# menonsamir/spiral

Measured on AMD Instinct MI355X. Metric: server ms/query + DB GB/s vs HBM roofline, 2^20 x 256B, lower is better.
Workload: dtype u32 residues, 32x32->64-bit integer MAC (two 28-bit CRT primes)

## Files before the change

### spiral_amd/csrc/digits_device.h

```cpp
#pragma once
#include <type_traits>

#include "common.h"
#include "ntt_device.h"

namespace spiral {

__device__ __forceinline__ uint64_t splitmix64(uint64_t x) {
    x += 0x9E3779B97F4A7C15ull;
    x = (x ^ (x >> 30)) * 0xBF58476D1CE4E5B9ull;
    x = (x ^ (x >> 27)) * 0x94D049BB133111EBull;
    return x ^ (x >> 31);
}

__device__ __forceinline__ uint64_t load_raw(const uint64_t* src, uint32_t idx, uint32_t tinv) {
    if (tinv == 0) return src[idx];
    uint32_t e = (idx * tinv) & (2 * kN - 1);
    uint64_t v = src[e & (kN - 1)];
    return (e & kN) ? kQ - v : v;
}

__device__ __forceinline__ uint64_t digit_of(uint64_t v, uint32_t k, uint32_t bits, uint64_t mask) {
    uint32_t sh = k * bits;
    if (bits <= 27u) {
// ... 12 lines not shown
    } else if (sh >= 32u) {
#pragma unroll
        for (int r = 0; r < 8; r++) d[r] = (hi32(raw[r]) >> (sh - 32u)) & mask;
    } else {
#pragma unroll
        for (int r = 0; r < 8; r++) d[r] = __builtin_amdgcn_alignbit(hi32(raw[r]), lo32(raw[r]), sh) & mask;
    }
}
__device__ __forceinline__ uint32_t udiv_small(uint32_t b, uint32_t d, uint32_t inv) { return d == 1u ? b : __umulhi(b, inv); }

template <bool SMALL>
__device__ __forceinline__ uint32_t digit_residue(uint32_t d, uint32_t m) {
    if constexpr (SMALL) return d;
    return d < (1u << 28) ? d : d % m;
}
constexpr uint32_t kSmallDigitBits = 27;
#define DIGIT_WIDTH_DISPATCH(bits, body) \
    do {                                 \
        if ((bits) <= kSmallDigitBits)   \
            body(std::true_type{});      \
        else                             \
            body(std::false_type{});     \
    } while (0)

struct SDigit {
    uint32_t sh_chain, sh_digit;
    uint64_t low_mask, thresh_in;
    uint64_t mask, base, thresh;
    bool has_in, may;
};
__device__ __forceinline__ SDigit sdigit_setup(uint32_t k, uint32_t bits, uint32_t ell) {
    SDigit d;
    const uint32_t half = ell >> 1, start = k < half ? 0u : half, j = k - start;
    d.base = 1ull << bits;
    d.mask = d.base - 1;
    d.thresh = d.base >> 1;
    d.sh_chain = start * bits;
    d.sh_digit = k * bits;
    d.has_in = j > 0;
    d.low_mask = (bits * j >= 64) ? ~0ull : ((1ull << (bits * j)) - 1);
    uint64_t t = 0;
    for (uint32_t i = 0; i < j; i++) t = (t << bits) + d.thresh;
    d.thresh_in = t;
    d.may = k < half ? (k + 1 < half) : true;
    return d;
}
// ... 139 lines not shown
```

### spiral_amd/csrc/kernels.h

```cpp
#pragma once
#include <hip/hip_runtime.h>
#include <stdint.h>
#include <stdlib.h>

#include <atomic>

#include "common.h"

namespace spiral {

struct IndexMap {
    uint32_t inner, outer_stride, off;
    __host__ __device__ uint32_t operator()(uint32_t b) const { return (b / inner) * outer_stride + (b % inner) + off; }
};
inline IndexMap identity_map() { return IndexMap{1u, 1u, 0u}; }

#ifdef SPIRAL_TUNING
inline const char* tuning_env(const char* name) { return getenv(name); }
#else
inline const char* tuning_env(const char*) { return nullptr; }
#endif
struct Options {
    int fold_pair = 1, fold_chain = 1, fwd2 = -1;
    uint32_t fold_blocks = 768, sweep_mfma_min = 2, fwd2_min = 8192;
    size_t db_stage_bytes = (size_t)64 << 20;
    int one_image = 1;
    uint32_t pack_item_group = 0;
    uint32_t pack_batch_lanes = 0;
    int pack_pair_blocks = 0;
    int sweep_narrow = 0;
    uint32_t query_batch_chunk = 512;
};
Options& options();

#ifndef SPIRAL_MAX_LANES
#define SPIRAL_MAX_LANES 8
#endif
constexpr uint32_t kMaxLanes = SPIRAL_MAX_LANES;
struct Lanes {
    uint32_t n = 1;
    int64_t off[kMaxLanes] = {};
#ifdef __HIPCC__
    __device__ __forceinline__ int64_t here() const {
        const uint32_t z = blockIdx.z;
        int64_t o = 0;
#pragma unroll
        for (uint32_t q = 1; q < kMaxLanes; q++) o = z == q ? off[q] : o;
        return o;
    }
    __device__ __forceinline__ int64_t at(int64_t stride) const { return (int64_t)blockIdx.z * stride; }
#endif
};
#ifdef __HIPCC__
// ... 228 lines not shown
void launch_response_wire_slots(const uint64_t* in, uint64_t* out, uint32_t n0, uint32_t w0, uint32_t n1, uint32_t w1, const Slots& slots, int64_t out_stride,
                                hipStream_t s);

struct ExpandMacParamsCore {
    uint64_t* cv;
    const uint64_t* w_e;
    const uint64_t* w_o;
    const uint64_t* g;
    const uint64_t* a1;
    uint32_t cnt_e, cnt_o, t_e, t_o;
    ExpandActive act;
    const uint64_t* neg1n;
    const uint64_t* neg1ns;
    uint32_t next_num_in, next_cnt_o;
};
template <class L>
struct ExpandMacParamsT : ExpandMacParamsCore {
    using Core = ExpandMacParamsCore;
    using NoLanesT = ExpandMacParamsT<NoLanes>;
    L lanes;
};
using ExpandMacParams = ExpandMacParamsT<Lanes>;
void launch_expand_mac_round(const ExpandMacParams& p, hipStream_t s);
struct Scal2MatParamsCore {
    const uint64_t* w;
    const uint64_t* g;
    const uint64_t* cv;
    IndexMap cv_pos;
    uint64_t* out;
    uint32_t* qs;
    uint32_t t_conv, count, jm_total, j_base;
};
template <class L>
struct Scal2MatParamsT : Scal2MatParamsCore {
    using Core = Scal2MatParamsCore;
    using NoLanesT = Scal2MatParamsT<NoLanes>;
    L lanes;
};
using Scal2MatParams = Scal2MatParamsT<Lanes>;
void launch_scal2mat(const Scal2MatParams& p, hipStream_t s);
struct GswParamsCore {
    const uint64_t* w;
    const uint64_t* v;
    const uint64_t* chat;
    const uint64_t* cv;
    IndexMap cv_pos;
// ... 244 lines not shown
```

### spiral_amd/csrc/ntt.hip

```cpp
#include <algorithm>
#include <cstdio>
#include <cstdlib>
#include <type_traits>

#include "digits_device.h"
#include "kernels.h"
#include "ntt_device.h"
#include "wire_device.h"

namespace spiral {

__device__ __forceinline__ void pk_load8_red(const uint64_t* poly, bool reduce, uint32_t tid, uint32_t* lo, uint32_t* hi) {
    uint64_t x[8];
    pk_load8(poly, tid, x);
    pk_unpack8(x, lo, hi);
    if (reduce) {
#pragma unroll
        for (int r = 0; r < 8; r++) {
            lo[r] %= kP;
            hi[r] %= kB;
        }
    }
}

// ... 46 lines not shown
                *p.err = 1u;
                v %= p.p_db;
            }
            if (v >= half_p) {
                uint64_t d = p.p_db - v;
                lo[r] = kP - mod_p(d);
                hi[r] = kB - mod_b(d);
            } else {
                lo[r] = mod_p(v);
                hi[r] = mod_b(v);
            }
        }
    } else if constexpr (LOAD == LD_PDIGIT) {
        uint32_t sp;
        if (p.pmode == PM_GSW) {
            sp = s;
        } else if (p.pmode == PM_FOLD) {
            const uint32_t per_t = 4u * p.fold_np, t = s / per_t, rem = s - t * per_t;
            sp = (t * p.pk_num_per + (rem >> 1)) * 2u + (rem & 1u);
        } else {
            sp = s * p.pk_num_per * 2u;
        }
        const uint64_t* src = p.src + (size_t)sp * kN;
        const uint64_t mask = (1ull << p.bits) - 1;
        uint64_t raw[8];
#pragma unroll
        for (int r = 0; r < 8; r++) raw[r] = src[ix_a(tid, r)];
        if (p.bits <= kSmallDigitBits) {
            udigits8(raw, k, p.bits, lo);
#pragma unroll
            for (int r = 0; r < 8; r++) hi[r] = lo[r];
        } else {
#pragma unroll
            for (int r = 0; r < 8; r++) {
                uint32_t d = (uint32_t)digit_of(raw[r], k, p.bits, mask);
                lo[r] = digit_residue<false>(d, kP);
                hi[r] = digit_residue<false>(d, kB);
            }
        }
    } else if constexpr (LOAD == LD_EXPAND) {
        const uint32_t je = p.cnt_e * p.t_e;
        uint32_t a, tdim;
        if (b < je) {
            tdim = p.t_e;
            a = udiv_small(b, tdim, p.inv_te);
            k = b - a * tdim;
        } else {
            tdim = p.t_o;
            const uint32_t bb = b - je;
            a = udiv_small(bb, tdim, p.inv_to);
            k = bb - a * tdim;
            a += p.cnt_e;
        }
        const uint64_t* src = p.src + (size_t)a * 2u * kN;
        uint64_t raw[8];
#pragma unroll
        for (int r = 0; r < 8; r++) raw[r] = src[ix_a(tid, r)];
        const uint32_t bits = get_bits_per(tdim);
        if (bits <= kSmallDigitBits) {
            udigits8(raw, k, bits, lo);
#pragma unroll
            for (int r = 0; r < 8; r++) hi[r] = lo[r];
        } else {
            const uint64_t mask = (1ull << bits) - 1;
#pragma unroll
            for (int r = 0; r < 8; r++) {
                const uint32_t d = (uint32_t)digit_of(raw[r], k, bits, mask);
                lo[r] = digit_residue<false>(d, kP);
                hi[r] = digit_residue<false>(d, kB);
            }
        }
        s = b;
    } else if constexpr (LOAD == LD_SDIFF) {
        const uint32_t i = s / 6u, rc = s - i * 6u;
        const uint64_t* sl = p.src + ((size_t)i * 6u + rc) * kN;
        const uint64_t* sh_ = p.src + ((size_t)(p.fold_np + i) * 6u + rc) * kN;
        const SFast f = sfast_setup(k, p.bits, p.ell);
        if (f.ok && (!f.chain1 || f.x_hi)) {
            const uint32_t* wl = reinterpret_cast<const uint32_t*>(sl) + (f.chain1 ? 1u : 0u);
            const uint32_t* wh = reinterpret_cast<const uint32_t*>(sh_) + (f.chain1 ? 1u : 0u);
            uint32_t xl[8], xh[8];
#pragma unroll
            for (int r = 0; r < 8; r++) {
                xl[r] = wl[2u * ix_a(tid, r)];
                xh[r] = wh[2u * ix_a(tid, r)];
            }
            const uint32_t xs = f.chain1 ? f.x_sh : 0u;
            if (f.last0) {
#pragma unroll
                for (int r = 0; r < 8; r++) signed_residues((int32_t)(sfast_word<true>(xh[r], f) - sfast_word<true>(xl[r], f)), lo[r], hi[r]);
            } else if (xs == 0u) {
#pragma unroll
                for (int r = 0; r < 8; r++) signed_residues((int32_t)(sfast_word<false>(xh[r], f) - sfast_word<false>(xl[r], f)), lo[r], hi[r]);
            } else {
// ... 570 lines not shown
```

### spiral_amd/csrc/poly.hip

```cpp
#include <cstdlib>
#include <type_traits>
#include "common.h"
#include "kernels.h"

namespace spiral {

__device__ __forceinline__ uint32_t shoup32(uint32_t y, uint32_t w, uint32_t ws, uint32_t m) { return w * y - __umulhi(y, ws) * m; }

constexpr uint32_t kTpb = 256;
constexpr uint32_t kBpp = kN / kTpb;

struct Acc2 {
    uint64_t lo = 0, hi = 0;
    __device__ __forceinline__ void mac(uint64_t a, uint64_t b) {
        lo += (uint64_t)lo32(a) * lo32(b);
        hi += (uint64_t)hi32(a) * hi32(b);
    }
    __device__ __forceinline__ uint64_t reduced() const { return pack(mod_p(lo), mod_b(hi)); }
};
__device__ __forceinline__ uint64_t add_pk(uint64_t a, uint64_t b) {
    return pack(csub(lo32(a) + lo32(b), kP), csub(hi32(a) + hi32(b), kB));
}

template <class L>
__global__ __launch_bounds__(kTpb) void matmul_kernel(MatmulParamsT<L> p) {
    const uint32_t z = blockIdx.x * kTpb + threadIdx.x;
    uint32_t rc = blockIdx.y, bt = blockIdx.z;
    if constexpr (!std::is_same<L, NoLanes>::value) {
        const int64_t lane = p.lanes.here();
        lane_shift(p.a, lane);
        lane_shift(p.b, lane);
        lane_shift(p.out, lane);
        bt = blockIdx.y / (p.rs * p.cs);
        rc = blockIdx.y - bt * (p.rs * p.cs);
    }
    const uint32_t r = rc / p.cs, c = rc - r * p.cs;
    const uint64_t* a = p.a + ((size_t)bt * p.a_batch + (size_t)r * p.ms) * kN + z;
    const uint64_t* b = p.b + ((size_t)bt * p.b_batch + c) * kN + z;
    Acc2 acc;
    for (uint32_t m = 0; m < p.ms; m++) acc.mac(a[(size_t)m * kN], b[(size_t)m * p.cs * kN]);
    p.out[((size_t)bt * p.out_batch + rc) * kN + z] = acc.reduced();
}
void launch_matmul(const MatmulParams& p, uint32_t batch, hipStream_t s) {
    if (batch == 0) return;
    if (p.lanes.n > 1)
// ... 1000 lines not shown
```

### spiral_amd/csrc/primitives.cpp

```cpp
#include "server_state.h"

thread_local std::string spiral::host::g_err;
std::atomic<uint64_t> spiral::host::g_pack_lane_batches{0};
std::atomic<uint64_t> spiral::g_mfma_sweeps{0};
std::atomic<uint64_t> spiral::host::g_db_export_ns{0};

spiral::Options& spiral::options() {
    static Options o = [] {
        Options v;
        if (const char* e = getenv("SPIRAL_FOLD_PAIR")) v.fold_pair = atoi(e) != 0;
        if (const char* e = getenv("SPIRAL_SWEEP_MFMA")) v.sweep_mfma_min = (uint32_t)strtoul(e, nullptr, 10);
        if (const char* e = getenv("SPIRAL_DB_STAGE_BYTES")) v.db_stage_bytes = (size_t)strtoull(e, nullptr, 10);
        return v;
    }();
    return o;
}

namespace {
size_t base_message_bytes(const spiral_gpu_params* p, MessageLayout (*layout)(const spiral_gpu_params&, const spiral_gpu_shape&), Form form) {
    spiral_gpu_shape s;
    return shape_of(p, &s) ? 0 : message_bytes(layout(*p, s), form);
}
}

extern "C" {

int spiral_gpu_abi_version(void) { return SPIRAL_GPU_ABI_VERSION; }

int spiral_gpu_set_option(const char* name, int64_t value) {
    if (!name) return fail("null option name");
    Options& o = options();
    const std::string n = name;
    if (n == "fold_pair") o.fold_pair = value != 0;
    else if (n == "fold_chain") o.fold_chain = value != 0;
    else if (n == "fold_blocks" && value >= 0) o.fold_blocks = (uint32_t)value;
    else if (n == "sweep_mfma_min" && value >= 0) o.sweep_mfma_min = (uint32_t)value;
    else if (n == "one_image") o.one_image = value != 0;
    else if (n == "fwd2" && value >= -1 && value <= 1) o.fwd2 = (int)value;
    else if (n == "fwd2_min" && value >= 0) o.fwd2_min = (uint32_t)value;
    else if (n == "db_stage_bytes" && value > 0) o.db_stage_bytes = (size_t)value;
    else if (n == "pack_item_group" && value >= 0 && value <= 0xFFFFFFFFll) o.pack_item_group = (uint32_t)value;
    else if (n == "pack_batch_lanes" && value >= 0 && value <= (int64_t)kMaxLanes) o.pack_batch_lanes = (uint32_t)value;
    else if (n == "pack_pair_blocks" && (value == 0 || value == 1)) o.pack_pair_blocks = (int)value;
    else if (n == "sweep_narrow" && (value == 0 || value == 1)) o.sweep_narrow = (int)value;
    else if (n == "query_batch_chunk" && value >= 1 && value <= 0xFFFFFFFFll) o.query_batch_chunk = (uint32_t)value;
    else return fail("unknown option '%s' or value %lld out of range", name, (long long)value);
    return 0;
}
int spiral_gpu_get_option(const char* name, int64_t* value) {
    if (!name || !value) return fail("null argument");
    const Options& o = options();
    const std::string n = name;
    if (n == "fold_pair") *value = o.fold_pair;
    else if (n == "fold_chain") *value = o.fold_chain;
    else if (n == "fold_blocks") *value = o.fold_blocks;
    else if (n == "sweep_mfma_min") *value = o.sweep_mfma_min;
    else if (n == "one_image") *value = o.one_image;
    else if (n == "fwd2") *value = o.fwd2;
    else if (n == "fwd2_min") *value = o.fwd2_min;
    else if (n == "db_stage_bytes") *value = (int64_t)o.db_stage_bytes;
    else if (n == "pack_item_group") *value = o.pack_item_group;
    else if (n == "pack_batch_lanes") *value = o.pack_batch_lanes;
    else if (n == "pack_pair_blocks") *value = o.pack_pair_blocks;
    else if (n == "sweep_narrow") *value = o.sweep_narrow;
    else if (n == "query_batch_chunk") *value = o.query_batch_chunk;
    else if (n == "graph_captures") *value = (int64_t)g_captures.load();
    else if (n == "pack_lane_batches") *value = (int64_t)g_pack_lane_batches.load();
    else if (n == "key_binds") *value = (int64_t)g_key_binds.load();
    else if (n == "db_export_ns") *value = (int64_t)g_db_export_ns.load();
    else if (n == "mfma_sweeps") *value = (int64_t)g_mfma_sweeps.load(std::memory_order_relaxed);
    else return fail("unknown option '%s'", name);
    return 0;
}
const char* spiral_gpu_last_error(void) { return g_err.c_str(); }
int spiral_gpu_device_count(void) {
    int n = 0;
    if (hipGetDeviceCount(&n) != hipSuccess) return 0;
    return n;
}
int spiral_gpu_get_shape(const spiral_gpu_params* p, spiral_gpu_shape* out) { return shape_of(p, out); }
int spiral_gpu_has_limb_form(const spiral_gpu_params* p, uint32_t j_begin, uint32_t j_end) {
    if (!p) return fail("null argument");
    spiral_gpu_shape s;
    spiral_gpu_params q = *p;
    q.direct_upload = 1;
    if (shape_of(&q, &s)) return -1;
    if (j_end == 0 && j_begin == 0) j_end = s.dim0;
    if (j_begin >= j_end || j_end > s.dim0) return fail("bad first-dimension shard [%u, %u) of %u", j_begin, j_end, s.dim0);
    return DbLayout::base(s.num_per, j_end - j_begin).limbs_ok() ? 1 : 0;
}
int spiral_gpu_column_shard_has_limb_form(const spiral_gpu_params* p, uint32_t n_ranks) {
    if (!p) return fail("null argument");
    spiral_gpu_shape s;
// ... 428 lines not shown
```

### spiral_amd/csrc/server.cpp

```cpp
#include "records_host.h"
#include "server_state.h"

std::atomic<uint64_t> spiral::host::g_captures{0};

namespace {

uint32_t fold_dpb(const spiral_gpu_server* S, uint32_t n_src) {
    uint32_t dpb = S->s.ell;
    while (dpb > 1 && n_src * ((S->s.ell + dpb - 1) / dpb) < S->fold_blocks) dpb = (dpb + 1) / 2;
    return dpb;
}

int srv_alloc(spiral_gpu_server* S, DbImage* owners) {
    const spiral_gpu_params& p = S->p;
    const spiral_gpu_shape& s = S->s;
    S->img = owners ? owners->share() : DbImage::create(DbLayout::base(srv_np(S), S->dim0_shard), S);
    if (!S->img) return -1;
    S->n_cv = p.direct_upload ? s.n_bits : (1u << s.g);
    const size_t ngs = (size_t)p.nu2 * s.ell;
    const size_t half = s.num_per > 1 ? s.num_per / 2 : 1;
    auto layout = [&](Arena& a) {
        a.carve(S->w_left, (size_t)s.n_left * 2 * p.t_exp * kN);
        a.carve(S->w_right, (size_t)s.n_right * 2 * p.t_exp_right * kN);
        a.carve(S->w, (size_t)3 * 2 * p.t_conv * kN);
// ... 162 lines not shown
    if (n_ii == 0 || ii0 >= S->s.num_per || n_ii > S->s.num_per - ii0) return fail("column range out of bounds");
    const size_t per_z = (size_t)n_ii * 2 * S->dim0_shard * 2;
    const uint32_t zchunk = (uint32_t)std::max<size_t>(1, std::min<size_t>(nz, ((size_t)256 << 20) / (per_z * sizeof(uint64_t))));
    DevBuf st;
    if (st.alloc(per_z * zchunk)) return -1;
    hipError_t e = hipSuccess;
    for (uint32_t z = 0; z < nz && e == hipSuccess; z += zchunk) {
        const uint32_t n = std::min(zchunk, nz - z);
        launch_db_read_slots(S->img->db.p, st.p, S->s.num_per, S->dim0_shard, z_begin + z, n, ii0, n_ii, S->stream, S->img->format == SPIRAL_GPU_DB_LIMBS);
        e = hipMemcpyAsync(out + (size_t)z * per_z, st.p, (size_t)n * per_z * sizeof(uint64_t), hipMemcpyDeviceToHost, S->stream);
        if (e == hipSuccess) e = hipStreamSynchronize(S->stream);
    }
    st.release();
    if (e != hipSuccess) return fail("database read-back failed: %s", hipGetErrorString(e));
    return 0;
}
}

namespace spiral {
namespace host {

void srv_check_epoch(spiral_gpu_server* S) {
    const uint64_t e = S->img->epoch;
    if (S->epoch_seen != e) {
        srv_drop_graphs(S);
        S->epoch_seen = e;
    }
}

int sweep_mfma(const uint64_t* limbs, const uint32_t* const* qs, uint64_t* const* acc, uint32_t n, uint32_t np, uint32_t jm, uint32_t g_log, hipStream_t st,
               uint32_t k_log, uint32_t g_extra) {
    const hipError_t e = launch_sweep_mfma(limbs, qs, acc, n, np, jm, g_log, st, k_log, g_extra);
    return e == hipSuccess ? 0 : fail("the matrix-core sweep could not be launched: %s", hipGetErrorString(e));
}
int sweep_one(spiral_gpu_server* S, int stage) {
    const DbImage* H = S->img;
    if (H->format == SPIRAL_GPU_DB_LIMBS) {
        if (stage >= 0 && S->sweep_k_log)
            return fail("a staged sweep needs the packed database image, and a batch has since converted it to limb planes: call set_sweep_stages again (or set option one_image = 0)");
        const uint32_t* qs[1] = {(const uint32_t*)S->qs.p};
        uint64_t* acc[1] = {S->acc};
        return sweep_mfma(H->db.p, qs, acc, 1, srv_np(S), 2 * S->dim0_shard, sweep_g_log(S), S->stream, S->sweep_k_log);
    }
    launch_sweep(H->db.p, (const uint32_t*)S->qs.p, S->acc, srv_np(S), 2 * S->dim0_shard, sweep_g_log(S), S->stream, S->sweep_k_log, stage);
    return 0;
}

int srv_join_side(spiral_gpu_server* S) {
    if (S->side_pending) {
        HIP_OK(hipStreamWaitEvent(S->stream, S->ev_join, 0));
// ... 4 lines not shown

void mark_raw_stale(spiral_gpu_server* const* servers, uint32_t n) {
    for (uint32_t b = 0; b < n; b++) servers[b]->raw_from_acc = false;
}
void mark_swept(spiral_gpu_server* const* servers, uint32_t n) {
    for (uint32_t b = 0; b < n; b++) servers[b]->have_records = true;
    mark_raw_stale(servers, n);
}

int expand_lanes(spiral_gpu_server* S, const Lanes& lanes, uint32_t r_begin, uint32_t r_end) {
    const spiral_gpu_params& p = S->p;
    if (p.direct_upload || S->s.g == 0) {
        const size_t n = p.direct_upload ? (size_t)S->s.n_bits * 2 : 2;
        for (uint32_t q = 0; q < lanes.n && r_begin == 0; q++)
            HIP_OK(hipMemcpyAsync(S->cv.p + lanes.off[q], S->query.p + lanes.off[q], n * kPolyBytes, hipMemcpyDeviceToDevice, S->stream));
        return 0;
    }
    ExpandWork wk{S->ex_raw.p, S->ex_g.p};
    run_expand(S->tb, S->cv.p, S->s.g, p.t_exp, S->w_left.p, p.t_exp_right, S->w_right.p, S->s.ell * p.nu2, S->s.stopround, wk, S->stream, S->query.p, r_begin, r_end,
               S->ex_shard, 3, lanes);
    return 0;
}

int convert_part(spiral_gpu_server* S, uint32_t what, hipStream_t st, bool mark_split, const Lanes& lanes) {
    const spiral_gpu_params& p = S->p;
    const spiral_gpu_shape& s = S->s;
    const uint32_t ps = S->pos_stride, ngs = p.nu2 * s.ell;
    if (ngs == 0) what &= ~CONV_GSW;
    if (what & CONV_S2M) S->have_records = true;
    const uint32_t n1 = (what & CONV_S2M) ? S->dim0_shard : 0, n2 = (what & CONV_GSW) ? 2 * ngs : 0;
    const IndexMap map1{1, 2 * ps, 2 * (S->j0 * ps + S->pos_first)};
    const IndexMap map2{2, 2 * ps, 2 * S->pos_rest};
    uint64_t* raw = n1 ? S->cv_raw.p : S->gs_raw_p;
    launch_job(S->tb, lift_job(S->cv.p, raw, n1 + n2, {.src_map = n1 ? map1 : map2, .split = (n1 && n2) ? n1 : 0, .src_map2 = map2, .lanes = lanes}), st);
    launch_job(S->tb, gadget_digits_job(raw, n1 ? S->cv_g.p : S->gs_chat_p, n1 + n2, p.t_conv, 2 * p.t_conv, lanes), st);
    Scal2MatParams sp{};
    sp.w = S->w.p;
    sp.g = S->cv_g.p;
    sp.cv = S->cv.p;
    sp.cv_pos = IndexMap{1, ps, S->j0 * ps + S->pos_first};
    sp.out = S->keep_cts ? S->cts_keep.p : nullptr;
    sp.qs = (uint32_t*)S->qs.p;
    sp.t_conv = p.t_conv;
    sp.count = S->dim0_shard;
    sp.jm_total = 2 * S->dim0_shard;
    sp.j_base = 0;
    sp.lanes = lanes;
    GswParams gp{};
    gp.w = S->w.p;
    gp.v = S->v.p;
    gp.chat = S->gs_chat_p;
    gp.cv = S->cv.p;
    gp.cv_pos = IndexMap{1, ps, S->pos_rest};
    gp.gsw = S->key.p;
    gp.t_conv = p.t_conv;
    gp.ell = s.ell;
    gp.dims = p.nu2;
    gp.key = nullptr;
    gp.lanes = lanes;
    if (what == CONV_BOTH && !mark_split) {
        launch_convert_products(sp, gp, st);
        return 0;
    }
    if (what & CONV_S2M) launch_scal2mat(sp, st);
    if (mark_split) HIP_OK(hipEventRecord(S->ev[7], st));
    if (what & CONV_GSW) launch_regev_to_gsw(gp, st);
    return 0;
}

int expand_convert(spiral_gpu_server* S) {
    if (expand_lanes(S, Lanes{})) return -1;
    return convert_part(S, CONV_BOTH, S->stream, !S->use_graphs);
}

int finish_lanes(spiral_gpu_server* S, const Lanes& lanes) {
    launch_rescale2(S->raw.p, S->resp.p, 2 * kN, 6 * kN, kQ, S->s.qprime, 4 * S->p.p_db, S->stream, lanes);
    return 0;
}
int run_fold_rounds(spiral_gpu_server* S, const FoldJob& job) {
    const spiral_gpu_shape& s = S->s;
    const Lanes& lanes = job.lanes;
    S->raw_from_acc = false;
    uint32_t np = job.np0;
    const uint64_t *src_pk = job.src_pk, *raw_addend = job.raw_addend;
    bool pre_reduce = job.pre_reduce;
    auto lift = [&](uint32_t npolys) {
        launch_job(S->tb, lift_job(src_pk, S->raw.p, npolys, {.pre_reduce = pre_reduce, .lanes = lanes}), S->stream);
        src_pk = nullptr;
    };
    auto digits = [&](FwdLoad ld, uint32_t n_src, uint32_t mac_terms) {
        launch_job(S->tb, fold_digits_job(ld, S->raw.p, S->fold_d.p, n_src, s.ell, np, mac_terms, lanes), S->stream);
    };
    uint64_t* out_pk = S->fold_c.p;
    for (uint32_t d = job.d0; d < job.d0 + job.rounds; d++) {
        np /= 2;
// ... 555 lines not shown
}

int spiral_gpu_server_run_pre(spiral_gpu_server* S) {
    if (enter(S)) return -1;
    if (!S->have_query || !S->have_pp) return fail("query and public parameters must be set first");
    const spiral_gpu_params& p = S->p;
    auto half = [&](uint32_t parity, hipStream_t st, uint64_t* raw, uint64_t* g) {
        ExpandWork wk{raw, g};
        run_expand(S->tb, S->cv.p, S->s.g, p.t_exp, S->w_left.p, p.t_exp_right, S->w_right.p, S->s.ell * p.nu2, S->s.stopround, wk, st, S->query.p, 0, 0xffffffffu,
                   ExpandShard{}, parity);
    };
    if (S->overlap) {
        if (srv_join_side(S)) return -1;
        HIP_OK(hipEventRecord(S->ev_fork, S->stream));
        HIP_OK(hipStreamWaitEvent(S->side_stream, S->ev_fork, 0));
        if (run_graph(S, G_PRE_SIDE, S->side_stream, {}, [&]() {
                half(2u, S->side_stream, S->ex_raw2.p, S->ex_g2.p);
                return convert_part(S, CONV_GSW, S->side_stream);
            }))
            return -1;
        HIP_OK(hipEventRecord(S->ev_join, S->side_stream));
        S->side_pending = true;
    }
    if (int rc = run_graph(S, G_PRE, S->stream, {}, [&]() {
            if (!S->overlap) return expand_convert(S);
            half(1u, S->stream, S->ex_raw.p, S->ex_g.p);
            return convert_part(S, CONV_S2M, S->stream);
        }))
        return rc;
    S->have_records = true;
    return 0;
}

int spiral_gpu_server_run_query(spiral_gpu_server* S) {
    if (enter(S)) return -1;
    if (refuse_column(S, "run_query")) return -1;
    if (!S->have_query || !S->have_pp) return fail("query and public parameters must be set first");
    if (!S->img->loaded) return fail("no database loaded");
    if (S->overlap) {
        if (spiral_gpu_server_run_pre(S)) return -1;
        if (spiral_gpu_server_first_dim(S)) return -1;
        return spiral_gpu_server_run_post(S, 0);
    }
    if (srv_join_side(S)) return -1;
    if (int rc = run_graph(S, G_QUERY, S->stream, {}, [&]() {
            if (expand_convert(S)) return -1;
            if (spiral_gpu_server_first_dim(S)) return -1;
            return run_fold_rounds(S, {.np0 = S->s.num_per, .rounds = S->p.nu2, .src_pk = S->acc, .finish = true});
        }))
        return rc;
    mark_swept(&S, 1);
    return 0;
}

int spiral_gpu_server_fold_local(spiral_gpu_server* S, const void* acc_chunk, void* out_ct) {
    if (!S || !acc_chunk || !out_ct) return fail("null argument");
    if (refuse_column(S, "fold_local")) return -1;
    HIP_OK(hipSetDevice(S->device));
    const uint32_t L = S->s.num_per >> S->fold_g_log;
    if (srv_join_side(S)) return -1;
    if (int rc = run_graph(S, G_FOLD_LOCAL, S->stream, {word(acc_chunk), word(out_ct)}, [&]() {
            if (run_fold_rounds(S, {.np0 = L, .rounds = S->p.nu2 - S->fold_g_log, .src_pk = (const uint64_t*)acc_chunk, .pre_reduce = true})) return -1;
            HIP_OK(hipMemcpyAsync(out_ct, S->raw.p, 6 * kPolyBytes, hipMemcpyDeviceToDevice, S->stream));
            return 0;
        }))
        return rc;
    S->raw_from_acc = false;
    return 0;
}

int spiral_gpu_server_fold_root(spiral_gpu_server* S, const void* gathered_cts) {
    if (!S || !gathered_cts) return fail("null argument");
    HIP_OK(hipSetDevice(S->device));
    const uint32_t G = 1u << S->fold_g_log;
    if (srv_join_side(S)) return -1;
    if (int rc = run_graph(S, G_FOLD_ROOT, S->stream, {word(gathered_cts)}, [&]() {
            HIP_OK(hipMemcpyAsync(S->raw.p, gathered_cts, (size_t)G * 6 * kPolyBytes, hipMemcpyDeviceToDevice, S->stream));
            return run_fold_rounds(S, {.np0 = G, .d0 = S->p.nu2 - S->fold_g_log, .rounds = S->fold_g_log, .finish = true});
        }))
        return rc;
    S->raw_from_acc = false;
    return 0;
}

int spiral_gpu_server_run_pre_sweep(spiral_gpu_server* S) {
    if (enter(S)) return -1;
    if (refuse_column(S, "run_pre_sweep")) return -1;
    if (!S->have_query || !S->have_pp) return fail("query and public parameters must be set first");
    if (!S->img->loaded) return fail("no database loaded");
    if (S->overlap) {
        if (spiral_gpu_server_run_pre(S)) return -1;
        return spiral_gpu_server_first_dim(S);
    }
    if (int rc = run_graph(S, G_PRE_SWEEP, S->stream, {}, [&]() {
            if (expand_convert(S)) return -1;
            return spiral_gpu_server_first_dim(S);
        }))
        return rc;
    mark_swept(&S, 1);
    return 0;
}

int spiral_gpu_server_run_expand_pack(spiral_gpu_server* S, void* bits_out) {
    if (!S || !bits_out) return fail("null argument");
    if (refuse_column(S, "run_expand_pack")) return -1;
    HIP_OK(hipSetDevice(S->device));
    if (!S->have_query || !S->have_pp) return fail("query and public parameters must be set first");
    return run_graph(S, G_EXPAND_PACK, S->stream, {word(bits_out)}, [&]() {
        if (expand_lanes(S, Lanes{})) return -1;
        return spiral_gpu_server_gsw_bits_pack(S, bits_out);
    });
}

int spiral_gpu_server_run_unpack_convert_sweep(spiral_gpu_server* S, const void* gathered) {
    if (!S || !gathered) return fail("null argument");
    if (refuse_column(S, "run_unpack_convert_sweep")) return -1;
    HIP_OK(hipSetDevice(S->device));
    if (!S->img->loaded) return fail("no database loaded");
    if (int rc = run_graph(S, G_UNPACK_CONVERT_SWEEP, S->stream, {word(gathered)}, [&]() {
            if (spiral_gpu_server_gsw_bits_unpack(S, gathered)) return -1;
            if (convert_part(S, CONV_BOTH, S->stream, !S->use_graphs)) return -1;
// ... 216 lines not shown
```

### spiral_amd/csrc/server_lanes.cpp

```cpp
#include "server_state.h"

namespace {

int check_lanes(spiral_gpu_server* const* servers, uint32_t n, const char* what, uint32_t needs, Lanes* lanes) {
    const bool whole = !(needs & SWEEP_ONLY), sharded = needs & SHARDED, moves = needs & MOVES_DATA;
    const bool column_ok = needs & (COLUMN_SHARDS | COLUMN_ONLY | MOVES_DATA | GIVES_KEYS | SWEEP_ONLY);
    return check_lane_list(servers, n, what, needs, lanes, [&](uint32_t b) {
        const spiral_gpu_server *S = servers[0], *L = servers[b];
        if (L->col.on && !column_ok) return refuse_column(L, what);
        if ((needs & COLUMN_ONLY) && !L->col.on) return fail("%s: server %u is not a column shard (create_column_shard)", what, b);
        if (!(L->col == S->col))
            return fail("%s: server %u is %s, server 0 %s: the lanes of a call are column shards of one rank and rank count, or none is", what, b,
                        L->col.on ? "a column shard of another rank or rank count" : "no column shard", S->col.on ? "is a column shard" : "is none");
        if (whole && (((needs & NEED_QUERY) && !L->have_query) || (!L->have_pp && !(needs & (GIVES_KEYS | MOVES_DATA))))) return fail("%s: server %u needs its query and public parameters set first", what, b);
        if ((needs & NEED_DB) && !L->img->loaded) return fail("%s: server %u has no database", what, b);
        if ((needs & NEED_RECORDS) && !L->have_records) return fail("%s: server %u has not converted its query (run_pre first)", what, b);
        if (L->device != S->device || L->dim0_shard != S->dim0_shard || L->s.num_per != S->s.num_per ||
            (whole && (memcmp(&L->p, &S->p, sizeof(S->p)) != 0 || L->j0 != S->j0 || L->j1 != S->j1)))
            return fail("%s: server %u differs from server 0 in parameters, device or shard", what, b);
        if ((sharded || !whole) && L->fold_g_log != S->fold_g_log)
            return fail("%s: server %u has %u fold ranks, server 0 has %u", what, b, 1u << L->fold_g_log, 1u << S->fold_g_log);
        if (sharded && (L->ex_shard.g_log != S->ex_shard.g_log || L->ex_shard.rank != S->ex_shard.rank))
            return fail("%s: server %u has another expansion shard than server 0", what, b);
        if (whole && !sharded && !moves && (L->acc != L->acc_own.p || (L->fold_g_log && !L->col.on) || L->ex_shard.g_log))
// ... 347 lines not shown
            if (sweep_image(S->img, limbs, qs, acc, n, 0, S->stream)) return -1;
            return run_fold_rounds(S, {.np0 = S->s.num_per, .rounds = S->p.nu2, .src_pk = S->acc, .finish = true, .lanes = lanes});
        });
    if (!rc) mark_swept(servers, n);
    return rc;
}

int spiral_gpu_server_run_query_instances(spiral_gpu_server* S, spiral_gpu_server* const* instances, uint32_t n, int pre, void* responses, void* finals) {
    if (!S || !instances || n == 0 || !responses) return fail("null argument");
    Lanes one;
    if (check_lanes(&S, 1, "run_query_instances", NEED_QUERY | (pre ? 0 : NEED_RECORDS), &one)) return -1;
    if (check_instances(S, instances, n, "run_query_instances")) return -1;
    std::vector<uint64_t> key{word(responses), word(finals), pre != 0};
    key_instances(&key, instances, n, nullptr);
    if (srv_join_side(S)) return -1;
    ItemOut o;
    o.resp = (uint64_t*)responses;
    o.fin = (uint64_t*)finals;
    o.via_resp = true;
    auto body = [&]() {
        if (pre && expand_convert(S)) return -1;
        return item_rounds(&S, Lanes{}, instances, nullptr, n, o);
    };
    if (int rc = run_graph(S, G_INSTANCES, S->stream, key, body)) return rc;
    if (pre)
        mark_swept(&S, 1);
    else
        mark_raw_stale(&S, 1);
    return 0;
}

int spiral_gpu_server_answer_instances(spiral_gpu_server* S, spiral_gpu_server* const* instances, uint32_t n, const uint64_t* query, uint64_t* responses,
                                       uint64_t* finals, double* total_us) {
    if (!S || !instances || n == 0 || !query || !responses) return fail("null argument");
    if (refuse_column(S, "answer_instances")) return -1;
    HIP_OK(hipSetDevice(S->device));
    if (spiral_gpu_server_set_query(S, query)) return -1;
    const size_t bytes = (size_t)n * 6 * kPolyBytes;
    return answer_on_host(S, {responses, bytes}, {finals, bytes}, total_us,
                          [&](void* d_resp, void* d_fin) { return spiral_gpu_server_run_query_instances(S, instances, n, 1, d_resp, d_fin); });
}

int spiral_gpu_server_run_query_batch_instances(spiral_gpu_server* const* servers, uint32_t n, spiral_gpu_server* const* instances, uint32_t n_inst, int pre,
                                                void* responses, void* finals, void* wire) {
    Lanes lanes;
    if (!responses && !wire) return fail("run_query_batch_instances: no output (responses or wire)");
    if (check_batch_instances(servers, n, instances, n_inst, pre, true, &lanes)) return -1;
// ... 189 lines not shown
```

### spiral_amd/csrc/server_state.h

```cpp
#pragma once
#include "db_image.h"
#include "key_store.h"
#include "message.h"

using namespace spiral;
using namespace spiral::host;

enum GraphId : int {
    G_PRE = 0,
    G_POST = 1,
    G_POST_REDUCE = 2,
    G_PRE_SIDE = 3,
    G_QUERY = 4,
    G_FOLD_LOCAL = 5,
    G_FOLD_ROOT = 6,
    G_PRE_SWEEP = 7,
    G_EXPAND_PACK = 8,
    G_UNPACK_CONVERT_SWEEP = 9,
    G_SCAL2MAT_SWEEP = 10,
    G_UNPACK_GSW = 11,
    G_SCAL2MAT = 12,
    G_BATCH,
    G_INSTANCES,
    G_BATCH_INSTANCES,
// ... 32 lines not shown
    DevBuf w_left, w_right, w, v, query, cv, ex_raw, ex_g, ex_raw2, ex_g2;
    DevBuf cv_raw, cv_g, key, cts_keep;
    uint64_t *gs_raw_p = nullptr, *gs_chat_p = nullptr;
    DevBuf qs, acc_own, raw, fold_d, fold_c, fold_c2, resp, stage;
    WireIn wire_in;
    QueryBatchIn query_batch_in;
    KeyMemo key_memo;
    uint64_t* acc = nullptr;
    hipEvent_t ev[8] = {};
    bool use_graphs = false;
    Captured graphs[G_COUNT];
    int overlap = 0;
    bool side_pending = false;
    hipStream_t side_stream = nullptr;
    hipEvent_t ev_fork = nullptr, ev_join = nullptr;
    bool fold_chain = true;
    bool fold_pair = true;
    uint32_t fold_blocks = 768;
    uint32_t fold_g_log = 0;
    uint32_t sweep_k_log = 0;
    ExpandShard ex_shard{};
    uint32_t sweep_mfma_min = 2;
    uint64_t epoch_seen = 0;
};

namespace spiral {
namespace host {

extern std::atomic<uint64_t> g_captures;

struct FoldJob {
    uint32_t np0 = 0, d0 = 0, rounds = 0;
    const uint64_t* src_pk = nullptr;
    bool pre_reduce = false, finish = false;
    const uint64_t* raw_addend = nullptr;
    Lanes lanes{};
};
enum ConvertWhat : uint32_t { CONV_S2M = 1, CONV_GSW = 2, CONV_BOTH = 3 };

constexpr uint32_t kMinShardColumns = 1;
inline uint32_t column_shard_columns(uint32_t num_per, uint32_t rank, uint32_t n_ranks) {
    if (n_ranks == 0 || (n_ranks & (n_ranks - 1))) return fail("column shards: %u ranks, the rank count must be a power of two", n_ranks), 0u;
    if (num_per / n_ranks < kMinShardColumns)
        return fail("column shards: %u ranks leave %u of %u ciphertext columns per shard, a shard needs at least %u", n_ranks, num_per / n_ranks, num_per,
                    kMinShardColumns),
               0u;
    if (rank >= n_ranks) return fail("column shard %u of %u: no such rank", rank, n_ranks), 0u;
    return num_per / n_ranks;
}
inline uint32_t srv_np(const spiral_gpu_server* S) { return S->s.num_per >> (S->col.on ? S->col.g_log : 0u); }
inline uint32_t col_g_log(const spiral_gpu_server* S) { return S->col.on ? S->col.g_log : 0u; }
inline uint32_t col_ranks(const spiral_gpu_server* S) { return 1u << col_g_log(S); }
inline bool holds_column(const spiral_gpu_server* S, uint32_t ii) { return (ii & (col_ranks(S) - 1u)) == (S->col.on ? S->col.rank : 0u); }
inline uint32_t sweep_g_log(const spiral_gpu_server* S) { return S->col.on ? 0u : S->fold_g_log; }
inline int refuse_column(const spiral_gpu_server* S, const char* what) {
    if (S && S->col.on)
        return fail("%s: this server is a column shard (create_column_shard): it holds %u of %u ciphertext columns, so it answers through run_column_batch, "
                    "the all-gather and fold_root_batch only", what, srv_np(S), S->s.num_per);
    return 0;
}
void srv_check_epoch(spiral_gpu_server* S);
int srv_join_side(spiral_gpu_server* S);
void mark_raw_stale(spiral_gpu_server* const* servers, uint32_t n);
void mark_swept(spiral_gpu_server* const* servers, uint32_t n);
int sweep_mfma(const uint64_t* limbs, const uint32_t* const* qs, uint64_t* const* acc, uint32_t n, uint32_t np, uint32_t jm, uint32_t g_log, hipStream_t st,
               uint32_t k_log = 0, uint32_t g_extra = 0);
int sweep_one(spiral_gpu_server* S, int stage);
int expand_lanes(spiral_gpu_server* S, const Lanes& lanes, uint32_t r_begin = 0, uint32_t r_end = 0xffffffffu);
int convert_part(spiral_gpu_server* S, uint32_t what, hipStream_t st, bool mark_split = false, const Lanes& lanes = Lanes{});
int expand_convert(spiral_gpu_server* S);
int finish_lanes(spiral_gpu_server* S, const Lanes& lanes);
int run_fold_rounds(spiral_gpu_server* S, const FoldJob& job);

template <class One>
int sweep_queries(const uint64_t* db, const uint64_t* limbs, uint32_t np, uint32_t jm, const uint32_t* const* qs, uint64_t* const* acc, uint32_t n, uint32_t g_log,
                  hipStream_t st, uint32_t k_log, uint32_t g_extra, One one) {
    if (limbs) return sweep_mfma(limbs, qs, acc, n, np, jm, g_log, st, k_log, g_extra);
    const uint32_t step = sweep_batch_ok(np, jm) ? kSweepMaxBatch : 1;
    for (uint32_t b0 = 0; b0 < n; b0 += step) {
        const uint32_t nb = n - b0 < step ? n - b0 : step;
        if (nb > 1)
            launch_sweep_batch(db, qs + b0, acc + b0, nb, np, jm, g_log, st, g_extra);
        else if (int rc = one(b0))
            return rc;
    }
    return 0;
}
inline int sweep_queries(const uint64_t* db, const uint64_t* limbs, uint32_t np, uint32_t jm, const uint32_t* const* qs, uint64_t* const* acc, uint32_t n, uint32_t g_log,
                         hipStream_t st, uint32_t k_log = 0) {
    return sweep_queries(db, limbs, np, jm, qs, acc, n, g_log, st, k_log, 0, [&](uint32_t b) {
        launch_sweep(db, qs[b], acc[b], np, jm, g_log, st, k_log);
        return 0;
    });
// ... 47 lines not shown
```

Baseline: 0.7231.

## Fuse last query-expansion round with CRT lift and gadget digit conversion

Adds a single kernel that runs the final expansion round (inverse NTT, automorphism, digit decomposition, forward NTTs, key-switch MAC) and immediately lifts and gadget-decomposes each leaf for conversion, instead of separate expansion, lift and gadget-digit launches. This removes the intermediate global round-trips and extra launches for the leaf ciphertexts. It is enabled by default when the last round has at least 256 leaves and adds a large fused kernel with heavy LDS use and serial per-digit NTTs per block.

Result: faster. 0.7124 (median of 6 runs) (-1.5%).

```diff
diff --git a/spiral_amd/csrc/digits_device.h b/spiral_amd/csrc/digits_device.h
--- a/spiral_amd/csrc/digits_device.h
+++ b/spiral_amd/csrc/digits_device.h
@@ -58,6 +58,22 @@
         else                             \
             body(std::false_type{});     \
     } while (0)
+
+__device__ __forceinline__ void udigit_inputs8(const uint64_t* raw, uint32_t k, uint32_t bits, uint32_t* lo, uint32_t* hi) {
+    if (bits <= kSmallDigitBits) {
+        udigits8(raw, k, bits, lo);
+#pragma unroll
+        for (int r = 0; r < 8; r++) hi[r] = lo[r];
+    } else {
+        const uint64_t mask = (1ull << bits) - 1;
+#pragma unroll
+        for (int r = 0; r < 8; r++) {
+            const uint32_t d = (uint32_t)digit_of(raw[r], k, bits, mask);
+            lo[r] = digit_residue<false>(d, kP);
+            hi[r] = digit_residue<false>(d, kB);
+        }
+    }
+}
 
 struct SDigit {
     uint32_t sh_chain, sh_digit;
diff --git a/spiral_amd/csrc/kernels.h b/spiral_amd/csrc/kernels.h
--- a/spiral_amd/csrc/kernels.h
+++ b/spiral_amd/csrc/kernels.h
@@ -29,6 +29,8 @@
     uint32_t pack_batch_lanes = 0;
     int pack_pair_blocks = 0;
     int sweep_narrow = 0;
+    int leaf_fuse = 1;
+    uint32_t leaf_fuse_min = 256;
     uint32_t query_batch_chunk = 512;
 };
 Options& options();
@@ -303,6 +305,18 @@
 };
 using ExpandMacParams = ExpandMacParamsT<Lanes>;
 void launch_expand_mac_round(const ExpandMacParams& p, hipStream_t s);
+struct LeafParams {
+    uint64_t* cv;
+    const uint64_t* w_e;
+    uint64_t* conv_g;
+    uint32_t n_leaves, t_e, auto_t;
+    uint32_t j0, n_first;
+    uint32_t t_conv, conv_lazy;
+    uint32_t n_plain;
+    IndexMap plain_map;
+};
+void launch_expand_leaf(const DeviceTables& t, const LeafParams& p, hipStream_t s);
+extern std::atomic<uint64_t> g_leaf_launches;
 struct Scal2MatParamsCore {
     const uint64_t* w;
     const uint64_t* g;
diff --git a/spiral_amd/csrc/leaf.hip b/spiral_amd/csrc/leaf.hip
--- /dev/null
+++ b/spiral_amd/csrc/leaf.hip
@@ -0,0 +1,98 @@
+#include "digits_device.h"
+#include "kernels.h"
+#include "mac_device.h"
+#include "ntt_device.h"
+
+namespace spiral {
+
+__global__ __launch_bounds__(256, 2) void expand_leaf_kernel(Tables t, LeafParams p) {
+    __shared__ uint64_t sh[kLdsWords];
+    __shared__ uint64_t sh_a1[kN];
+    const uint32_t tid = threadIdx.x, b = blockIdx.x;
+    uint32_t lo[8], hi[8];
+    uint64_t raw[8];
+    uint32_t conv_dst;
+    if (b < p.n_leaves) {
+        const uint32_t a = b;
+        uint64_t* c = p.cv + (size_t)a * 4u * kN;
+        uint64_t v[8];
+        pk_load8(c, tid, v);
+        pk_unpack8(v, lo, hi);
+        uint64_t a1[8];
+#pragma unroll
+        for (int r = 0; r < 8; r++) {
+            const uint32_t e = ((2u * (__brev(8u * tid + r) >> 21) + 1u) * p.auto_t) & (2u * kN - 1u);
+            a1[r] = c[kN + pk_pos(__brev(e >> 1) >> 21)];
+        }
+        ntt_inverse_block<false>(lo, hi, sh, t.inv, tid);
+#pragma unroll
+        for (int r = 0; r < 8; r++) sh_a1[256u * r + tid] = a1[r];
+        __syncthreads();
+#pragma unroll
+        for (int r = 0; r < 8; r++) {
+            const uint32_t e = (ix_a(tid, r) * p.auto_t) & (2u * kN - 1u);
+            const uint64_t x = crt_compose_lazy(csub_min(lo[r], kP), hi[r]);
+            sh[lds_ix(e & (kN - 1u))] = (e & kN) ? kQ - x : x;
+        }
+        __syncthreads();
+#pragma unroll
+        for (int r = 0; r < 8; r++) raw[r] = sh[lds_ix(ix_a(tid, r))];
+        const uint32_t bits = get_bits_per(p.t_e);
+        Acc2 acc0[8], acc1[8];
+        for (uint32_t k = 0; k < p.t_e; k++) {
+            uint64_t w0[8], w1[8];
+            pk_load8(p.w_e + (size_t)k * kN, tid, w0);
+            pk_load8(p.w_e + (size_t)(p.t_e + k) * kN, tid, w1);
+            udigit_inputs8(raw, k, bits, lo, hi);
+            __syncthreads();
+            ntt_forward_block<false>(lo, hi, sh, t.fwd, tid);
+#pragma unroll
+            for (int r = 0; r < 8; r++) {
+                const uint64_t g = pack(lo[r], hi[r]);
+                acc0[r].mac(w0[r], g);
+                acc1[r].mac(w1[r], g);
+            }
+        }
+        uint64_t old1[8];
+        pk_load8(c, tid, v);
+        pk_load8(c + kN, tid, old1);
+#pragma unroll
+        for (int r = 0; r < 8; r++) {
+            v[r] = add_pk(v[r], acc0[r].reduced());
+            old1[r] = add_pk(add_pk(old1[r], acc1[r].reduced()), sh_a1[256u * r + tid]);
+        }
+        pk_store8(c, tid, v);
+        pk_store8(c + kN, tid, old1);
+        if (a - p.j0 >= p.n_first) return;
+        conv_dst = (a - p.j0) * p.t_conv;
+        pk_unpack8(v, lo, hi);
+        __syncthreads();
+    } else {
+        const uint32_t s = b - p.n_leaves;
+        conv_dst = (p.n_first + s) * p.t_conv;
+        uint64_t v[8];
+        pk_load8(p.cv + (size_t)p.plain_map(s) * kN, tid, v);
+        pk_unpack8(v, lo, hi);
+    }
+    ntt_inverse_block<false>(lo, hi, sh, t.inv, tid);
+    crt_lift8(lo, hi, raw);
+    const uint32_t cbits = get_bits_per(p.t_conv);
+    for (uint32_t k = 0; k < p.t_conv; k++) {
+        udigit_inputs8(raw, k, cbits, lo, hi);
+        __syncthreads();
+        ntt_forward_block<false>(lo, hi, sh, t.fwd, tid);
+        if (!p.conv_lazy) canonicalize8(lo, hi);
+        uint64_t x[8];
+        pk_pack8(lo, hi, x);
+        pk_store8(p.conv_g + (size_t)(conv_dst + k) * kN, tid, x);
+    }
+}
+
+void launch_expand_leaf(const DeviceTables& t, const LeafParams& p, hipStream_t s) {
+    if (p.n_leaves + p.n_plain == 0) return;
+    Tables tb{t.fwd, t.inv};
+    hipLaunchKernelGGL(expand_leaf_kernel, dim3(p.n_leaves + p.n_plain), dim3(256), 0, s, tb, p);
+    g_leaf_launches.fetch_add(1, std::memory_order_relaxed);
+}
+
+}
diff --git a/spiral_amd/csrc/mac_device.h b/spiral_amd/csrc/mac_device.h
--- /dev/null
+++ b/spiral_amd/csrc/mac_device.h
@@ -0,0 +1,20 @@
+#pragma once
+#include "common.h"
+
+namespace spiral {
+
+__device__ __forceinline__ uint32_t shoup32(uint32_t y, uint32_t w, uint32_t ws, uint32_t m) { return w * y - __umulhi(y, ws) * m; }
+
+struct Acc2 {
+    uint64_t lo = 0, hi = 0;
+    __device__ __forceinline__ void mac(uint64_t a, uint64_t b) {
+        lo += (uint64_t)lo32(a) * lo32(b);
+        hi += (uint64_t)hi32(a) * hi32(b);
+    }
+    __device__ __forceinline__ uint64_t reduced() const { return pack(mod_p(lo), mod_b(hi)); }
+};
+__device__ __forceinline__ uint64_t add_pk(uint64_t a, uint64_t b) {
+    return pack(csub(lo32(a) + lo32(b), kP), csub(hi32(a) + hi32(b), kB));
+}
+
+}
diff --git a/spiral_amd/csrc/ntt.hip b/spiral_amd/csrc/ntt.hip
--- a/spiral_amd/csrc/ntt.hip
+++ b/spiral_amd/csrc/ntt.hip
@@ -92,22 +92,10 @@
             sp = s * p.pk_num_per * 2u;
         }
         const uint64_t* src = p.src + (size_t)sp * kN;
-        const uint64_t mask = (1ull << p.bits) - 1;
         uint64_t raw[8];
 #pragma unroll
         for (int r = 0; r < 8; r++) raw[r] = src[ix_a(tid, r)];
-        if (p.bits <= kSmallDigitBits) {
-            udigits8(raw, k, p.bits, lo);
-#pragma unroll
-            for (int r = 0; r < 8; r++) hi[r] = lo[r];
-        } else {
-#pragma unroll
-            for (int r = 0; r < 8; r++) {
-                uint32_t d = (uint32_t)digit_of(raw[r], k, p.bits, mask);
-                lo[r] = digit_residue<false>(d, kP);
-                hi[r] = digit_residue<false>(d, kB);
-            }
-        }
+        udigit_inputs8(raw, k, p.bits, lo, hi);
     } else if constexpr (LOAD == LD_EXPAND) {
         const uint32_t je = p.cnt_e * p.t_e;
         uint32_t a, tdim;
@@ -126,20 +114,7 @@
         uint64_t raw[8];
 #pragma unroll
         for (int r = 0; r < 8; r++) raw[r] = src[ix_a(tid, r)];
-        const uint32_t bits = get_bits_per(tdim);
-        if (bits <= kSmallDigitBits) {
-            udigits8(raw, k, bits, lo);
-#pragma unroll
-            for (int r = 0; r < 8; r++) hi[r] = lo[r];
-        } else {
-            const uint64_t mask = (1ull << bits) - 1;
-#pragma unroll
-            for (int r = 0; r < 8; r++) {
-                const uint32_t d = (uint32_t)digit_of(raw[r], k, bits, mask);
-                lo[r] = digit_residue<false>(d, kP);
-                hi[r] = digit_residue<false>(d, kB);
-            }
-        }
+        udigit_inputs8(raw, k, get_bits_per(tdim), lo, hi);
         s = b;
     } else if constexpr (LOAD == LD_SDIFF) {
         const uint32_t i = s / 6u, rc = s - i * 6u;
diff --git a/spiral_amd/csrc/poly.hip b/spiral_amd/csrc/poly.hip
--- a/spiral_amd/csrc/poly.hip
+++ b/spiral_amd/csrc/poly.hip
@@ -2,25 +2,12 @@
 #include <type_traits>
 #include "common.h"
 #include "kernels.h"
+#include "mac_device.h"
 
 namespace spiral {
-
-__device__ __forceinline__ uint32_t shoup32(uint32_t y, uint32_t w, uint32_t ws, uint32_t m) { return w * y - __umulhi(y, ws) * m; }
 
 constexpr uint32_t kTpb = 256;
 constexpr uint32_t kBpp = kN / kTpb;
-
-struct Acc2 {
-    uint64_t lo = 0, hi = 0;
-    __device__ __forceinline__ void mac(uint64_t a, uint64_t b) {
-        lo += (uint64_t)lo32(a) * lo32(b);
-        hi += (uint64_t)hi32(a) * hi32(b);
-    }
-    __device__ __forceinline__ uint64_t reduced() const { return pack(mod_p(lo), mod_b(hi)); }
-};
-__device__ __forceinline__ uint64_t add_pk(uint64_t a, uint64_t b) {
-    return pack(csub(lo32(a) + lo32(b), kP), csub(hi32(a) + hi32(b), kB));
-}
 
 template <class L>
 __global__ __launch_bounds__(kTpb) void matmul_kernel(MatmulParamsT<L> p) {
diff --git a/spiral_amd/csrc/primitives.cpp b/spiral_amd/csrc/primitives.cpp
--- a/spiral_amd/csrc/primitives.cpp
+++ b/spiral_amd/csrc/primitives.cpp
@@ -3,6 +3,7 @@
 thread_local std::string spiral::host::g_err;
 std::atomic<uint64_t> spiral::host::g_pack_lane_batches{0};
 std::atomic<uint64_t> spiral::g_mfma_sweeps{0};
+std::atomic<uint64_t> spiral::g_leaf_launches{0};
 std::atomic<uint64_t> spiral::host::g_db_export_ns{0};
 
 spiral::Options& spiral::options() {
@@ -44,6 +45,8 @@
     else if (n == "pack_pair_blocks" && (value == 0 || value == 1)) o.pack_pair_blocks = (int)value;
     else if (n == "sweep_narrow" && (value == 0 || value == 1)) o.sweep_narrow = (int)value;
     else if (n == "query_batch_chunk" && value >= 1 && value <= 0xFFFFFFFFll) o.query_batch_chunk = (uint32_t)value;
+    else if (n == "leaf_fuse" && (value == 0 || value == 1)) o.leaf_fuse = (int)value;
+    else if (n == "leaf_fuse_min" && value >= 0 && value <= 0xFFFFFFFFll) o.leaf_fuse_min = (uint32_t)value;
     else return fail("unknown option '%s' or value %lld out of range", name, (long long)value);
     return 0;
 }
@@ -64,11 +67,14 @@
     else if (n == "pack_pair_blocks") *value = o.pack_pair_blocks;
     else if (n == "sweep_narrow") *value = o.sweep_narrow;
     else if (n == "query_batch_chunk") *value = o.query_batch_chunk;
+    else if (n == "leaf_fuse") *value = o.leaf_fuse;
+    else if (n == "leaf_fuse_min") *value = o.leaf_fuse_min;
     else if (n == "graph_captures") *value = (int64_t)g_captures.load();
     else if (n == "pack_lane_batches") *value = (int64_t)g_pack_lane_batches.load();
     else if (n == "key_binds") *value = (int64_t)g_key_binds.load();
     else if (n == "db_export_ns") *value = (int64_t)g_db_export_ns.load();
     else if (n == "mfma_sweeps") *value = (int64_t)g_mfma_sweeps.load(std::memory_order_relaxed);
+    else if (n == "leaf_launches") *value = (int64_t)g_leaf_launches.load(std::memory_order_relaxed);
     else return fail("unknown option '%s'", name);
     return 0;
 }
diff --git a/spiral_amd/csrc/server.cpp b/spiral_amd/csrc/server.cpp
--- a/spiral_amd/csrc/server.cpp
+++ b/spiral_amd/csrc/server.cpp
@@ -208,10 +208,23 @@
 
 void srv_check_epoch(spiral_gpu_server* S) {
     const uint64_t e = S->img->epoch;
-    if (S->epoch_seen != e) {
+    const bool leaf = leaf_fused(S);
+    if (S->epoch_seen != e || S->leaf_seen != leaf) {
         srv_drop_graphs(S);
         S->epoch_seen = e;
-    }
+        S->leaf_seen = leaf;
+    }
+}
+
+bool leaf_fused(const spiral_gpu_server* S) {
+    const Options& o = options();
+    const spiral_gpu_shape& s = S->s;
+    if (!o.leaf_fuse || S->p.direct_upload || s.g == 0 || s.stopround == 0 || s.g - 1 <= s.stopround) return false;
+    if (S->ex_shard.g_log || S->overlap || S->p.nu2 * s.ell == 0) return false;
+    return (1u << (s.g - 1)) >= o.leaf_fuse_min;
+}
+void count_leaf_replay(const spiral_gpu_server* S, uint64_t before) {
+    if (leaf_fused(S) && g_leaf_launches.load(std::memory_order_relaxed) == before) g_leaf_launches.fetch_add(1, std::memory_order_relaxed);
 }
 
 int sweep_mfma(const uint64_t* limbs, const uint32_t* const* qs, uint64_t* const* acc, uint32_t n, uint32_t np, uint32_t jm, uint32_t g_log, hipStream_t st,
@@ -262,7 +275,7 @@
     return 0;
 }
 
-int convert_part(spiral_gpu_server* S, uint32_t what, hipStream_t st, bool mark_split, const Lanes& lanes) {
+int convert_part(spiral_gpu_server* S, uint32_t what, hipStream_t st, bool mark_split, const Lanes& lanes, bool leaf_round) {
     const spiral_gpu_params& p = S->p;
     const spiral_gpu_shape& s = S->s;
     const uint32_t ps = S->pos_stride, ngs = p.nu2 * s.ell;
@@ -271,9 +284,28 @@
     const uint32_t n1 = (what & CONV_S2M) ? S->dim0_shard : 0, n2 = (what & CONV_GSW) ? 2 * ngs : 0;
     const IndexMap map1{1, 2 * ps, 2 * (S->j0 * ps + S->pos_first)};
     const IndexMap map2{2, 2 * ps, 2 * S->pos_rest};
-    uint64_t* raw = n1 ? S->cv_raw.p : S->gs_raw_p;
-    launch_job(S->tb, lift_job(S->cv.p, raw, n1 + n2, {.src_map = n1 ? map1 : map2, .split = (n1 && n2) ? n1 : 0, .src_map2 = map2, .lanes = lanes}), st);
-    launch_job(S->tb, gadget_digits_job(raw, n1 ? S->cv_g.p : S->gs_chat_p, n1 + n2, p.t_conv, 2 * p.t_conv, lanes), st);
+    if (leaf_round) {
+        if (what != CONV_BOTH || lanes.n != 1 || ps != 2 || S->pos_first != 0) return fail("the fused leaf round needs one query's whole conversion in the reordered layout");
+        const uint32_t r = s.g - 1;
+        LeafParams lp{};
+        lp.cv = S->cv.p;
+        lp.w_e = S->w_left.p + (size_t)r * 2 * p.t_exp * kN;
+        lp.conv_g = S->cv_g.p;
+        lp.n_leaves = 1u << r;
+        lp.t_e = p.t_exp;
+        lp.auto_t = (kN >> r) + 1;
+        lp.j0 = S->j0;
+        lp.n_first = n1;
+        lp.t_conv = p.t_conv;
+        lp.conv_lazy = gadget_digits_job(nullptr, nullptr, 0, p.t_conv, 2 * p.t_conv).p.lazy_out;
+        lp.n_plain = n2;
+        lp.plain_map = map2;
+        launch_expand_leaf(S->tb, lp, st);
+    } else {
+        uint64_t* raw = n1 ? S->cv_raw.p : S->gs_raw_p;
+        launch_job(S->tb, lift_job(S->cv.p, raw, n1 + n2, {.src_map = n1 ? map1 : map2, .split = (n1 && n2) ? n1 : 0, .src_map2 = map2, .lanes = lanes}), st);
+        launch_job(S->tb, gadget_digits_job(raw, n1 ? S->cv_g.p : S->gs_chat_p, n1 + n2, p.t_conv, 2 * p.t_conv, lanes), st);
+    }
     Scal2MatParams sp{};
     sp.w = S->w.p;
     sp.g = S->cv_g.p;
@@ -309,8 +341,9 @@
 }
 
 int expand_convert(spiral_gpu_server* S) {
-    if (expand_lanes(S, Lanes{})) return -1;
-    return convert_part(S, CONV_BOTH, S->stream, !S->use_graphs);
+    const bool leaf = leaf_fused(S);
+    if (expand_lanes(S, Lanes{}, 0, leaf ? S->s.g - 1 : 0xffffffffu)) return -1;
+    return convert_part(S, CONV_BOTH, S->stream, !S->use_graphs, Lanes{}, leaf);
 }
 
 int finish_lanes(spiral_gpu_server* S, const Lanes& lanes) {
@@ -912,12 +945,14 @@
         HIP_OK(hipEventRecord(S->ev_join, S->side_stream));
         S->side_pending = true;
     }
+    const uint64_t leaf0 = g_leaf_launches.load(std::memory_order_relaxed);
     if (int rc = run_graph(S, G_PRE, S->stream, {}, [&]() {
             if (!S->overlap) return expand_convert(S);
             half(1u, S->stream, S->ex_raw.p, S->ex_g.p);
             return convert_part(S, CONV_S2M, S->stream);
         }))
         return rc;
+    count_leaf_replay(S, leaf0);
     S->have_records = true;
     return 0;
 }
@@ -933,12 +968,14 @@
         return spiral_gpu_server_run_post(S, 0);
     }
     if (srv_join_side(S)) return -1;
+    const uint64_t leaf0 = g_leaf_launches.load(std::memory_order_relaxed);
     if (int rc = run_graph(S, G_QUERY, S->stream, {}, [&]() {
             if (expand_convert(S)) return -1;
             if (spiral_gpu_server_first_dim(S)) return -1;
             return run_fold_rounds(S, {.np0 = S->s.num_per, .rounds = S->p.nu2, .src_pk = S->acc, .finish = true});
         }))
         return rc;
+    count_leaf_replay(S, leaf0);
     mark_swept(&S, 1);
     return 0;
 }
@@ -982,11 +1019,13 @@
         if (spiral_gpu_server_run_pre(S)) return -1;
         return spiral_gpu_server_first_dim(S);
     }
+    const uint64_t leaf0 = g_leaf_launches.load(std::memory_order_relaxed);
     if (int rc = run_graph(S, G_PRE_SWEEP, S->stream, {}, [&]() {
             if (expand_convert(S)) return -1;
             return spiral_gpu_server_first_dim(S);
         }))
         return rc;
+    count_leaf_replay(S, leaf0);
     mark_swept(&S, 1);
     return 0;
 }
diff --git a/spiral_amd/csrc/server_lanes.cpp b/spiral_amd/csrc/server_lanes.cpp
--- a/spiral_amd/csrc/server_lanes.cpp
+++ b/spiral_amd/csrc/server_lanes.cpp
@@ -393,7 +393,9 @@
         if (pre && expand_convert(S)) return -1;
         return item_rounds(&S, Lanes{}, instances, nullptr, n, o);
     };
+    const uint64_t leaf0 = g_leaf_launches.load(std::memory_order_relaxed);
     if (int rc = run_graph(S, G_INSTANCES, S->stream, key, body)) return rc;
+    if (pre) count_leaf_replay(S, leaf0);
     if (pre)
         mark_swept(&S, 1);
     else
diff --git a/spiral_amd/csrc/server_state.h b/spiral_amd/csrc/server_state.h
--- a/spiral_amd/csrc/server_state.h
+++ b/spiral_amd/csrc/server_state.h
@@ -78,6 +78,7 @@
     ExpandShard ex_shard{};
     uint32_t sweep_mfma_min = 2;
     uint64_t epoch_seen = 0;
+    bool leaf_seen = false;
 };
 
 namespace spiral {
@@ -123,8 +124,10 @@
                uint32_t k_log = 0, uint32_t g_extra = 0);
 int sweep_one(spiral_gpu_server* S, int stage);
 int expand_lanes(spiral_gpu_server* S, const Lanes& lanes, uint32_t r_begin = 0, uint32_t r_end = 0xffffffffu);
-int convert_part(spiral_gpu_server* S, uint32_t what, hipStream_t st, bool mark_split = false, const Lanes& lanes = Lanes{});
+int convert_part(spiral_gpu_server* S, uint32_t what, hipStream_t st, bool mark_split = false, const Lanes& lanes = Lanes{}, bool leaf_round = false);
 int expand_convert(spiral_gpu_server* S);
+bool leaf_fused(const spiral_gpu_server* S);
+void count_leaf_replay(const spiral_gpu_server* S, uint64_t before);
 int finish_lanes(spiral_gpu_server* S, const Lanes& lanes);
 int run_fold_rounds(spiral_gpu_server* S, const FoldJob& job);
 
```
